# knram06/multigrid_parallel

Hardware: AMD Instinct MI355X
Metric: V-cycles/sec, 513^3 ('512^3') Poisson, V(2,2), fp64 (higher is better)
Workload: dtype f64

## Files before the change

### multigrid_parallel_amd/csrc/mg3d_ctx.hip

```cpp
#include "mg3d_ctx.h"

#include <math.h>
#include <stdarg.h>
#include <stdio.h>
#include <stdlib.h>
#include <string.h>

#include <algorithm>
#include <vector>

static thread_local char g_err[512] = "";

int mg3d_fail(int code, const char *fmt, ...)
{
    va_list ap;
    va_start(ap, fmt);
    vsnprintf(g_err, sizeof g_err, fmt, ap);
    va_end(ap);
    return code;
}
#define fail mg3d_fail

int mg3d_alloc_fail(hipError_t e, const char *who, const char *what)
{
// ... 156 lines not shown
    if (ctx->dep_acc)
        (void)hipFree(ctx->dep_acc);
    if (ctx->dep_max)
        (void)hipFree(ctx->dep_max);
    if (ctx->push_table)
        (void)hipFree(ctx->push_table);
    if (ctx->sort_buf)
        (void)hipFree(ctx->sort_buf);
    for (hipEvent_t e : ctx->io_ev)
        if (e)
            (void)hipEventDestroy(e);
    if (ctx->dz_map)
        (void)hipFree(ctx->dz_map);
    if (ctx->partials)
        (void)hipFree(ctx->partials);
    if (ctx->sumsq)
        (void)hipFree(ctx->sumsq);
    if (ctx->h_sumsq)
        (void)hipHostFree(ctx->h_sumsq);
    resolve_timers(ctx);
    for (hipEvent_t e : ctx->event_pool)
        (void)hipEventDestroy(e);
    if (ctx->stream && ctx->own_stream)
        (void)hipStreamDestroy(ctx->stream);
    delete ctx;
    return MG3D_OK;
}

struct OptionRow {
    const char *key, *env;
    int mode;
    int dflt;
};
static const OptionRow kOptionTable[MG3D_OPT_COUNT] = {
    {"carry", "MG3D_NO_CARRY", 1, 1},
    {"carry_min", "MG3D_CARRY_MIN", 0, 130},
    {"legs", "MG3D_LEGS", 0, 1},
    {"legs_min", "MG3D_LEGS_MIN", 0, 160},
    {"tiny", "MG3D_NO_TINY", 1, 1},
    {"tiny_cycle", "MG3D_NO_TINY_CYCLE", 1, 1},
    {"lu_reduced", "MG3D_LU_REDUCED", 0, 1},
    {"fuse_rst2", "MG3D_FUSE_RST2", 0, -1},
    {"small_max", "MG3D_SMALL_MAX", 0, 129},
    {"fuse_leg_max", "MG3D_FUSE_LEG_MAX", 0, 0},
    {"fuse_up_max", "MG3D_FUSE_UP_MAX", 0, 1 << 20},
    {"sweep_tune", "MG3D_SWEEP_TUNE", 0, -1},
    {"sweep_tune_log", "MG3D_SWEEP_TUNE_LOG", 0, 0},
    {"sweep_ci", "MG3D_SWEEP_CI", 0, 0},
    {"sweep_rj", "MG3D_SWEEP_CFG", 2, 0},
    {"sweep_nw", nullptr, 0, 0},
    {"sweep_pf", nullptr, 0, 0},
    {"d_zero_skip", "MG3D_D_ZERO_SKIP", 0, 1},
    {"zero_front", "MG3D_ZERO_FRONT", 0, 1},
};

void mg3d_options_init(mg3d_options *o)
{
    for (int i = 0; i < MG3D_OPT_COUNT; i++) {
        const OptionRow &r = kOptionTable[i];
        o->v[i] = r.dflt;
        const char *e = r.env ? getenv(r.env) : nullptr;
        if (!e || !e[0])
            continue;
        if (r.mode == 0)
            o->v[i] = atoi(e);
        else if (r.mode == 1)
            o->v[i] = e[0] == '1' ? 0 : 1;
        else {
            int rj = 0, nw = 0, pf = 0;
            if (sscanf(e, "%d,%d,%d", &rj, &nw, &pf) >= 2) {
                o->v[MG3D_OPT_SWEEP_RJ] = rj;
                o->v[MG3D_OPT_SWEEP_NW] = nw;
                o->v[MG3D_OPT_SWEEP_PF] = pf;
            }
            i += 2;
        }
    }
}

int mg3d_option_index(const char *key)
{
    if (key)
        for (int i = 0; i < MG3D_OPT_COUNT; i++)
            if (strcmp(key, kOptionTable[i].key) == 0)
                return i;
    return -1;
}

const char *mg3d_option_key(int index) { return index >= 0 && index < MG3D_OPT_COUNT ? kOptionTable[index].key : nullptr; }

extern "C" const char *mg3d_option_name(int index) { return mg3d_option_key(index); }

static mg3d_ctx *ctx_new(int L, int iters)
{
    mg3d_ctx *ctx = new mg3d_ctx();
    ctx->c = 0;
    ctx->length = 0.;
    ctx->L = L;
    ctx->iters = iters;
    ctx->have_lu = false;
    ctx->sigma = 0.;
    ctx->lu_built = false;
    ctx->lu_h = 0.;
    ctx->periodic = 0;
    ctx->neumann = 0;
    ctx->per_b = nullptr;
// ... 513 lines not shown
{
    if (!ctx || !launches)
        return fail(MG3D_ERR_ARG, "mg3d_ctx_dnone_launches: NULL argument");
    *launches = ctx->dnone_launches;
    return MG3D_OK;
}

extern "C" int mg3d_ctx_sweep_taken(const mg3d_ctx *ctx, int kind, int which, int out[MG3D_SWEEP_TAKEN_FIELDS],
                                    unsigned long long *count, unsigned long long *launches)
{
    static_assert(sizeof(SweepTaken) == MG3D_SWEEP_TAKEN_FIELDS * sizeof(int), "SweepTaken is the MG3D_SWEEP_TAKEN_* fields in order");
    static_assert(MG3D_SWEEP_KIND_LEG_UP + 1 == MG3D_SWEEP_KINDS && MG3D_SWEEP_KIND_PASSES == SWEEP_PASSES &&
                      MG3D_SWEEP_KIND_PASSES_RES == SWEEP_PASSES_RES && MG3D_SWEEP_KIND_TAP == SWEEP_TAP &&
                      MG3D_SWEEP_KIND_LEG_DOWN == SWEEP_LEG_DOWN && MG3D_SWEEP_KIND_LEG_UP == SWEEP_LEG_UP,
                  "MG3D_SWEEP_KIND_* are SweepKind");
    if (!ctx || !out)
        return fail(MG3D_ERR_ARG, "mg3d_ctx_sweep_taken: NULL argument");
    if (kind < 0 || kind >= MG3D_SWEEP_KINDS || which < 0)
        return fail(MG3D_ERR_ARG, "mg3d_ctx_sweep_taken: no such kind, or a negative index");
    const SweepTakenLog &log = ctx->sweep_taken;
    const bool have = which < log.n[kind];
    if (have)
        memcpy(out, &log.e[kind][which].t, sizeof(SweepTaken));
    else
        memset(out, 0, sizeof(SweepTaken));
    if (count)
        *count = have ? log.e[kind][which].count : 0;
    if (launches)
        *launches = log.launches[kind];
    return MG3D_OK;
}

int mg3d_launch_ok(const char *who)
{
    hipError_t e = hipGetLastError();
    if (e != hipSuccess)
        return fail(MG3D_ERR_HIP, "%s: kernel launch failed: %s", who, hipGetErrorString(e));
    return MG3D_OK;
}

static int read_norm(mg3d_ctx *ctx, int slot, double *norm)
{
    if (!norm)
        return MG3D_OK;
    HIPCHK(hipMemcpyAsync(ctx->h_sumsq + slot, ctx->sumsq + slot, sizeof(double), hipMemcpyDeviceToHost,
                          ctx->stream));
    HIPCHK(hipStreamSynchronize(ctx->stream));
    resolve_timers(ctx);
    *norm = sqrt(ctx->h_sumsq[slot]);
    return MG3D_OK;
}

static StageAsk stage_ask(const mg3d_ctx *ctx, int level, int post, int iters, int want_res, bool has_coarse, bool need_norm,
                          bool pro_offered)
{
    const Geom &g = ctx->lv[level].g;
    return StageAsk{g.N, g.nj, post != 0, iters, want_res, has_coarse, need_norm, pro_offered,  true};
}

static int enqueue_stage_step(mg3d_ctx *ctx, int level, int post, const StageStep &st, bool first, int want_res, int slot,
                              Level *coarse, const Level *pro, bool zero_in, bool need_norm)
{
    Level &l = ctx->lv[level];
    SweepLaunch w = mg3d_level_sweep(ctx, l);
    w.kind = st.res ? SWEEP_PASSES_RES : SWEEP_PASSES;
    w.S = st.S;
    w.c1 = post ? 0 : 1;
    if (zero_in && first)
        w.vin = nullptr;
    if (st.res && want_res == 2 && !st.rst)
        w.r = l.f[MG3D_R];
    if (st.res && need_norm)
        w.partials = ctx->partials;
    if (st.rst) {
        w.gc = &coarse->g;
        w.dc = coarse->f[MG3D_D];
    }
    if (st.pro) {
        w.gce = &pro->g;
        w.ec = pro->f[MG3D_U];
    }
    int np;
    {
        StageScope kt(ctx, level, st.S == 4 ? MG3D_K_SWEEP4 : st.S == 2 ? (st.res ? MG3D_K_SWEEP2_RES : MG3D_K_SWEEP2)
                                                                        : MG3D_K_RESIDUAL, true);
        np = k_sweep(ctx->opt, w, ctx->stream);
    }
    if (np < 0)
        return fail(MG3D_ERR_STATE, "fused sweep: no kernel for %d colour passes%s on level %d", st.S,
                    st.res ? " + residual" : "", level);
    if (st.S > 0)
        swap_u(l);
    if (st.res && need_norm)
        k_fold(ctx->partials, np, ctx->sumsq + slot, ctx->stream);
    return MG3D_OK;
}

static int enqueue_smooth_residual(mg3d_ctx *ctx, int level, int post, int iters, int want_res, int slot,
                                    Level *coarse = nullptr, const Level *pro = nullptr, bool zero_in = false,
                                    bool need_norm = true)
{
    Level &l = ctx->lv[level];
    hipStream_t s = ctx->stream;
    if (mg3d_fused(ctx)) {
        const StagePlan plan = mg3d_stage_plan(ctx->opt, stage_ask(ctx, level, post, iters, want_res, coarse != nullptr, need_norm,
                                                                   pro != nullptr));
        for (int k = 0; mg3d_stage_launch(plan, k); k++)
            CHK(enqueue_stage_step(ctx, level, post, *mg3d_stage_launch(plan, k), k == 0, want_res, slot, coarse, pro, zero_in, need_norm));
        return MG3D_OK;
    }
    const int c1 = post ? 0 : 1;
    const LevelOperator A = mg3d_level_operator(ctx, level);
    for (int it = 0; it < 2 * iters; it++) {
        StageScope kt(ctx, level, MG3D_K_COLOUR_PASS, true);
        k_smooth_color(l.g, l.f[MG3D_U], l.f[MG3D_D], A, c1 ^ (it & 1), s);
    }
    if (want_res) {
        StageScope kt(ctx, level, MG3D_K_RESIDUAL, true);
        k_residual(l.g, l.f[MG3D_U], l.f[MG3D_D], A, want_res == 2 ? l.f[MG3D_R] : nullptr, ctx->partials, ctx->sumsq + slot, s);
    }
    return MG3D_OK;
}

static bool pro_fusable(const mg3d_ctx *ctx, int iters, int want_res, int level)
{
    return mg3d_fused(ctx) && mg3d_stage_plan(ctx->opt, stage_ask(ctx, level, 1, iters, want_res, false, true, true)).step[0].pro;
}

static void enqueue_restrict(mg3d_ctx *ctx, int level, bool faces_only = false)
{
    const Level &lev = ctx->lv[level], &lc = ctx->lv[level - 1];
    k_restrict(lev.g, lev.f[MG3D_R], lc.g, lc.f[MG3D_D], mg3d_ctx_bc(ctx), ctx->stream, -1, -1, faces_only);
}

static void enqueue_prolong(mg3d_ctx *ctx, int level)
{
    const Level &lev = ctx->lv[level], &lc = ctx->lv[level - 1];
    k_prolong(lc.g, lc.f[MG3D_U], lev.g, lev.f[MG3D_U], mg3d_ctx_bc(ctx), ctx->stream, -1, -1, mg3d_level_operator(ctx, level).m);
}

static void enqueue_coarse_solve(mg3d_ctx *ctx, const double *rhs = nullptr ,
                                 bool own_values = false )
{
    Level &l0 = ctx->lv[0];
    if (!rhs)
        rhs = l0.f[MG3D_D];
    const int bc = mg3d_ctx_bc(ctx), pin = mg3d_ctx_pinned(ctx);
    const unsigned char *m = mg3d_level_operator(ctx, 0).m;
    if (m || ctx->periodic || (ctx->neumann && pin)) {
        k_coarse_rhs(l0.g, rhs, ctx->per_b, bc, pin, m, (ctx->L == 1 || own_values) ? l0.f[MG3D_U] : nullptr, ctx->stream);
        rhs = ctx->per_b;
    }
    k_lu_solve(ctx->lu, ctx->lu_in, l0.g, rhs, l0.f[MG3D_U], ctx->lu_work, ctx->stream);
    k_per_refresh(l0.g, l0.f[MG3D_U], bc, ctx->stream);
}

static int enqueue_smooth(mg3d_ctx *ctx, int level, int post, int iters)
{
    return enqueue_smooth_residual(ctx, level, post, iters, 0, 0);
// ... 833 lines not shown
```

### multigrid_parallel_amd/csrc/mg3d_dist.hip

```cpp
#include "mg3d_ctx.h"

#include <math.h>
#include <stdio.h>
#include <stdlib.h>
#include <string.h>

#include <rccl/rccl.h>

#include "mg3d_plan.h"

#define fail mg3d_fail
#define HIPCHK(call)                                                                                    \
    do {                                                                                                \
        hipError_t e_ = (call);                                                                         \
        if (e_ != hipSuccess)                                                                           \
            return fail(MG3D_ERR_HIP, "%s failed: %s (%s:%d)", #call, hipGetErrorString(e_), __FILE__, \
                        __LINE__);                                                                      \
    } while (0)
#define NCCLCHK(call)                                                                                    \
    do {                                                                                                 \
        ncclResult_t e_ = (call);                                                                        \
        if (e_ != ncclSuccess)                                                                           \
            return fail(MG3D_ERR_HIP, "%s failed: %s (%s:%d)", #call, ncclGetErrorString(e_), __FILE__, \
                        __LINE__);                                                                       \
// ... 858 lines not shown
                HIPCHK(hipEventRecord(D->ev_now, xs));
                HIPCHK(hipStreamWaitEvent(s, D->ev_now, 0));
            }
        } else
            HIPCHK(hipMemcpyAsync(R.gather, R.coarse->sumsq, sizeof(double), hipMemcpyDeviceToDevice, s));
    }
    hipLaunchKernelGGL(sum_in_order_kernel, dim3(1), dim3(64), 0, s, R.gather, D->P, D->d_norms + slot);
    return MG3D_OK;
}

struct RestrictTarget {
    const Geom *gc;
    double *dc;
    int lo, hi;
};
static void restrict_into(SweepLaunch &w, const RestrictTarget &t)
{
    w.gc = t.gc;
    w.dc = t.dc;
    w.ic_lo = t.lo;
    w.ic_hi = t.hi;
}

struct ProlongSource {
    const Geom *gc;
    const double *ec;
};
static void prolong_from(SweepLaunch &w, const ProlongSource &p)
{
    w.gce = p.gc;
    w.ec = p.ec;
}

struct SlabCycle {
    int slot;
    bool carry_out, legs_out;
    bool carry_in, legs_in;
    bool red_in;
    bool can_legs, can_carry, keep_r;
};

struct Window {
    int lo, hi;
};
static Window slab_window(const SlabLevel &sl, int m)
{
    return Window{sl.own_lo - m < 0 ? 0 : sl.own_lo - m, sl.own_hi + m > sl.lv.g.ni ? sl.lv.g.ni : sl.own_hi + m};
}

static StagePlan dist_stage_plan(mg3d_dist *D, int l, int post, int want_res, bool has_coarse, bool pro_offered)
{
    const Geom &g = SL(D, D->rs[0], l).lv.g;
    return mg3d_stage_plan(D->rs[0].coarse->opt,
                           StageAsk{g.N, g.nj, post != 0, D->nu, want_res, has_coarse, want_res == 1, pro_offered,  false});
}

static SweepLaunch slab_sweep(mg3d_dist *D, size_t ri, int l)
{
    SlabLevel &sl = SL(D, D->rs[ri], l);
    SweepLaunch w = mg3d_level_sweep(D->rs[ri].coarse, sl.lv);
    w.i_lo = w.acc_lo = sl.own_lo;
    w.i_hi = w.acc_hi = sl.own_hi;
    return w;
}

static void swap_u_all(mg3d_dist *D, int l)
{
    for (auto &R : D->rs)
        swap_u(SL(D, R, l).lv);
}

template <class Make, class Done>
static int edge_first(mg3d_dist *D, int l, int margin, int E, const char *what, Make make, Done done)
{
    bool split = D->overlap && D->P > 1;
    std::vector<Window> win;
    for (auto &R : D->rs) {
        win.push_back(slab_window(SL(D, R, l), margin));
        split = split && win.back().hi - win.back().lo >= 2 * E + 2;
    }
    std::vector<int> n_first(D->rs.size());
    for (size_t ri = 0; ri < D->rs.size(); ri++) {
        SweepLaunch w = make(ri, split, -1);
        w.i_lo = win[ri].lo;
        w.i_hi = win[ri].hi;
        w.edge = split ? E : 0;
        n_first[ri] = k_sweep(D->rs[ri].coarse->opt, w, D->stream);
        if (n_first[ri] <= 0)
            return fail(MG3D_ERR_STATE, "slab sweep: no kernel for %s%s on level %d", split ? "the edge windows of " : "", what, l);
        if (!split)
            done(ri, n_first[ri], 0);
    }
    swap_u_all(D, l);
    CHK(start_u_exchange(D, MG3D_XK_HALO_U_NEXT, l));
    for (size_t ri = 0; split && ri < D->rs.size(); ri++) {
        Level &lv = SL(D, D->rs[ri], l).lv;
        SweepLaunch w = make(ri, split, n_first[ri]);
        w.vin = lv.alt;
        w.vout = lv.f[MG3D_U];
        w.i_lo = win[ri].lo + E;
        w.i_hi = win[ri].hi - E;
        const int n_in = k_sweep(D->rs[ri].coarse->opt, w, D->stream);
        if (n_in <= 0)
            return fail(MG3D_ERR_STATE, "slab sweep: no kernel for the interior window of %s on level %d", what, l);
        done(ri, n_first[ri], n_in);
    }
    return MG3D_OK;
// ... 394 lines not shown
```

### multigrid_parallel_amd/csrc/mg3d_internal.h

```cpp
#ifndef MG3D_INTERNAL_H
#define MG3D_INTERNAL_H

#include <hip/hip_runtime.h>
#include <stddef.h>

#include "mg3d.h"

struct Geom {
    int ni, nj, nk;
    int pitch;
    long long plane;
    int ig0;
    int N;
};

static inline int mg3d_pitch_for(int nk) { return (nk + 15) & ~15; }

struct LevelOp {
    double hSq, sixth, invHsq, dg;
};
static inline LevelOp mg3d_level_op(double h, double sigma)
{
    LevelOp op;
    op.hSq = h * h;
    op.dg = 6 + sigma * op.hSq;
    op.sixth = 1. / op.dg;
    op.invHsq = 1. / op.hSq;
    return op;
}

struct LuBand {
    int n;
    int bw;
    double *lcol;
    double *ucol;
    int npad;
    double *diag;
    int fast_div;
    int rot_r;
    double *lrot;
    double *urot;
    int stream_ch;
    double *stream;
    int *in_map;
};

#define MG3D_MAX_PARTIALS 32768

enum {
    MG3D_OPT_CARRY = 0,
    MG3D_OPT_CARRY_MIN,
    MG3D_OPT_LEGS,
    MG3D_OPT_LEGS_MIN,
    MG3D_OPT_TINY,
    MG3D_OPT_TINY_CYCLE,
    MG3D_OPT_LU_REDUCED,
    MG3D_OPT_FUSE_RST2,
    MG3D_OPT_SMALL_MAX,
    MG3D_OPT_FUSE_LEG_MAX,
    MG3D_OPT_FUSE_UP_MAX,
    MG3D_OPT_SWEEP_TUNE,
    MG3D_OPT_SWEEP_TUNE_LOG,
    MG3D_OPT_SWEEP_CI,
    MG3D_OPT_SWEEP_RJ,
    MG3D_OPT_SWEEP_NW,
    MG3D_OPT_SWEEP_PF,
    MG3D_OPT_D_ZERO_SKIP,
    MG3D_OPT_ZERO_FRONT,
    MG3D_OPT_COUNT
};
struct mg3d_options {
    int v[MG3D_OPT_COUNT];
};
void mg3d_options_init(mg3d_options *o);
int mg3d_option_index(const char *key);
const char *mg3d_option_key(int index);

struct LevelOperator {
    LevelOp op;
    double sigma;
    const double *e;
    int bc;
    const unsigned char *m;
    const double *s;
};
static inline int mg3d_bc(int periodic, int neumann) { return periodic | neumann << 3; }

void k_smooth_color(const Geom &g, double *v, const double *d, const LevelOperator &A, int color, hipStream_t s,
                    int i_lo = -1, int i_hi = -1);
void k_residual(const Geom &g, const double *v, const double *d, const LevelOperator &A, double *res, double *partials,
                double *sumsq_out, hipStream_t s, int i_lo = -1, int i_hi = -1, int acc_lo = 0, int acc_hi = -1);
void k_sumsq(const Geom &g, const double *a, double *partials, double *sumsq_out, hipStream_t s);
int k_pcg_apply_dot(const Geom &g, const double *p, const LevelOperator &A, double *q, double *partials, double *dot_out,
                    hipStream_t s);
int k_pcg_update_norm(const Geom &g, int bc, double *x, double *r, const double *p, const double *q, const double *rz,
                      const double *pap, double *partials, double *rr_out, hipStream_t s);
int k_pcg_dot(const Geom &g, int bc, const double *a, const double *b, double *partials, double *dot_out, hipStream_t s);
int k_pcg_direction(const Geom &g, int bc, double *p, const double *z, const double *rz_new, const double *rz_old,
                    hipStream_t s);
int k_wpcg_dot(const Geom &g, int bc, const double *a, const double *b, double *partials, double *dot_out, double *sum_out,
               hipStream_t s);
int k_wpcg_direction(const Geom &g, int bc, double *p, const double *z, const double *rz_new, const double *rz_old,
                     const double *wsum, double W, bool first, hipStream_t s);
int k_wpcg_center(const Geom &g, int bc, double *r, const double *wsum, double W, double *partials, double *rr_out,
                  hipStream_t s);
double k_wpcg_weight_sum(const Geom &g, int bc);
int k_step_rhs(const Geom &g, const double *u0, const double *src, const LevelOperator &A, double a, double c1, double b,
               bool backward_euler, double *d, hipStream_t s);
void k_restrict(const Geom &gf, const double *r, const Geom &gc, double *dc, int bc, hipStream_t s, int ic_lo = -1,
                int ic_hi = -1, bool faces_only = false ,
                const unsigned char *mf = nullptr );
void k_prolong(const Geom &gc, const double *ec, const Geom &gf, double *ef, int bc, hipStream_t s, int if_lo = -1,
               int if_hi = -1, const unsigned char *mf = nullptr );
void k_fill_boundary(const Geom &g, double *v, double h, hipStream_t s);
__host__ __device__ static inline int mg3d_dzero_words(int ni) { return (ni + 31) / 32; }
void k_dzero_scan(const Geom &g, const double *d, unsigned *map, hipStream_t s);
void k_dzero_fill(const Geom &g, unsigned *map, hipStream_t s);
void k_fold(const double *partials, int np, double *out, hipStream_t s);
void k_fold2(const double *pa, int na, const double *pb, int nb, double *out, hipStream_t s);
void k_sweep_set_tune_default(int on);
bool k_sweep_fuse_rst2(const mg3d_options &o, int N);
// ... 2 lines not shown
    SWEEP_PASSES_RES,
    SWEEP_TAP,
    SWEEP_LEG_DOWN,
    SWEEP_LEG_UP
};
struct SweepTaken {
    int S, RES, RJ, NW, PF, ND, DZ, CI, blocks, xcd_remap, ntj, ntk, PRO, RST, DP, TAP, N;
};
#define MG3D_SWEEP_KINDS 5
#define MG3D_SWEEP_TAKEN_KEEP 32
struct SweepTakenLog {
    struct Entry {
        SweepTaken t;
        unsigned long long count;
    };
    Entry e[MG3D_SWEEP_KINDS][MG3D_SWEEP_TAKEN_KEEP];
    int n[MG3D_SWEEP_KINDS];
    unsigned long long launches[MG3D_SWEEP_KINDS];
};
struct SweepLaunch {
    SweepTakenLog *taken = nullptr;
    const Geom *g = nullptr;
    LevelOp op = {};
    const double *vin = nullptr;
    const double *d = nullptr;
    const unsigned *d_zero = nullptr;
    bool d_none = false;
    unsigned long long *d_none_taken = nullptr;
    double *vout = nullptr;
    SweepKind kind = SWEEP_PASSES;
    int S = 0;
    int c1 = 1;
    double *r = nullptr;
    double *partials = nullptr;
    int max_partials = MG3D_MAX_PARTIALS;
    const Geom *gc = nullptr;
    double *dc = nullptr;
    int ic_lo = -1, ic_hi = -1;
    const Geom *gce = nullptr;
    const double *ec = nullptr;
    int i_lo = -1, i_hi = -1, acc_lo = 0, acc_hi = -1, edge = 0;
};
int k_sweep(const mg3d_options &o, const SweepLaunch &w, hipStream_t s);

struct StageAsk {
    int N, nj;
    bool post;
    int iters;
    int want_res;
    bool has_coarse;
    bool need_norm;
    bool pro_offered;
    bool leg4_form;
};
struct StageStep {
    int S;
    int times;
    bool res;
    bool rst;
    bool pro;
    bool last;
};
struct StagePlan {
    int n;
    StageStep step[3];
};
static inline StagePlan mg3d_stage_plan(const mg3d_options &o, const StageAsk &q)
{
    StagePlan p = {0, {}};
    const bool sp = q.post && 2 * q.iters == 4 && q.want_res == 1;
    const int up_max = q.leg4_form && o.v[MG3D_OPT_FUSE_LEG_MAX] > o.v[MG3D_OPT_FUSE_UP_MAX] ? o.v[MG3D_OPT_FUSE_LEG_MAX]
                                                                                              : o.v[MG3D_OPT_FUSE_UP_MAX];
    const bool pro = q.pro_offered && q.post &&
                     (sp || (2 * q.iters == 4 && q.want_res == 0 && (q.nj & 1) != 0 && q.N <= up_max));
    int passes = 2 * q.iters;
    bool done_res = q.want_res == 0;
    while (passes > 0 || !done_res) {
        const int S = (sp && passes >= 2) ? 2 : passes >= 4 ? 4 : passes;
        const bool last = passes - S == 0;
        const bool leg4 = q.leg4_form && S == 4 && q.has_coarse && !q.need_norm && q.want_res != 0 && q.N <= o.v[MG3D_OPT_FUSE_LEG_MAX];
        const bool res = last && q.want_res != 0 && (S != 4 || leg4) && !(S == 2 && q.has_coarse && !k_sweep_fuse_rst2(o, q.N));
        const StageStep st = {S, 1, res, res && q.has_coarse, pro && passes == 2 * q.iters, last};
        StageStep *prev = p.n ? &p.step[p.n - 1] : nullptr;
        if (prev && prev->S == S && !prev->res && !res && !prev->pro && prev->last == last)
            prev->times++;
        else if (p.n < 3)
            p.step[p.n++] = st;
        done_res = done_res || res;
        passes -= S;
    }
    return p;
}

static inline const StageStep *mg3d_stage_launch(const StagePlan &p, int k)
{
    for (int i = 0; i < p.n; k -= p.step[i++].times)
        if (k < p.step[i].times)
            return &p.step[i];
    return nullptr;
}

static inline bool mg3d_run_ahead_policy(const mg3d_options &o, bool legs, int N)
{
    return o.v[legs ? MG3D_OPT_LEGS : MG3D_OPT_CARRY] != 0 && N >= o.v[legs ? MG3D_OPT_LEGS_MIN : MG3D_OPT_CARRY_MIN];
}
static inline bool mg3d_can_run_ahead(const mg3d_options &o, bool legs, int forced, int iters, bool keep_r, int N, int nj)
{
    const bool on = forced >= 0 ? forced != 0 : mg3d_run_ahead_policy(o, legs, N);
    return on && iters == 2 && !keep_r && N > 65 && (nj & 1) != 0;
}
bool k_tiny_fits(const Geom &g, const Geom &gc);
void k_tiny_down(const Geom &g, double *u, const double *d, const double *r, const Geom &gc, double *dc, const LevelOp &op,
                 int iters, hipStream_t s);
void k_tiny_up(const Geom &g, double *u, const double *d, const Geom &gc, const double *ec, const LevelOp &op, int iters,
               hipStream_t s);
bool k_tiny_cycle_fits(const Geom &g, const Geom &gc, const LuBand &lu, const LuBand &lin);
void k_tiny_cycle(const Geom &g, double *u, const double *d, const double *r, const Geom &gc, double *dc, double *xc,
                  const LuBand &lu, const LuBand &lin, const LevelOp &op, int iters, hipStream_t s);
void k_coef_inject(const Geom &gf, const double *ef, const Geom &gc, double *ec, hipStream_t s);
void k_coarse_rhs(const Geom &g, const double *d, double *b, int bc, int pin, const unsigned char *m, const double *ufix,
                  hipStream_t s);
void k_per_refresh(const Geom &g, double *v, int bc, hipStream_t s, const unsigned long long *gate = nullptr);
void k_mask_pack(const Geom &g, unsigned char *m, const mg3d_array &a, int bc, hipStream_t s);
void k_mask_inject(const Geom &gf, const unsigned char *mf, const Geom &gc, unsigned char *mc, hipStream_t s);
void k_mask_refresh(const Geom &g, unsigned char *m, int bc, hipStream_t s);
void k_mask_keep(const Geom &gf, const unsigned char *mf, const Geom &gc, unsigned char *mc, hipStream_t s);
void k_mask_count(const Geom &g, const unsigned char *m, int bc, unsigned long long *out, hipStream_t s);
void k_fmg_interp(const Geom &gc, const double *uc, const Geom &gf, double *uf, int bc, hipStream_t s,
                  const unsigned char *mf = nullptr);
void k_fmg_inject(const Geom &gf, const double *uf, const unsigned char *mf, const Geom &gc, double *uc, int bc, hipStream_t s);
void k_dirichlet_rhs(const Geom &g, const double *u, double *d, int bc, hipStream_t s);
void k_zero_faces(const Geom &g, double *v, int faces, hipStream_t s);
void k_pack(const Geom &g, double *v, const mg3d_array &a, hipStream_t s);
void k_unpack(const Geom &g, const double *v, const mg3d_array &a, hipStream_t s);
// ... 33 lines not shown
```

### multigrid_parallel_amd/csrc/mg3d_sweep.hip

```cpp
#include "mg3d_internal.h"

#include <stdio.h>
#include <stdlib.h>
#include <string.h>

#include <algorithm>
#include <atomic>
#include <map>
#include <type_traits>
#include <mutex>
#include <vector>

#include "mg3d_sweep_kernel.h"

static std::atomic<int> g_sweep_tune_default{1};
void k_sweep_set_tune_default(int on) { g_sweep_tune_default.store(on); }

static int current_device()
{
    int dev = 0;
    (void)hipGetDevice(&dev);
    return dev;
}

static int device_cus()
{
    static std::mutex mu;
    static std::map<int, int> cus;
    const int dev = current_device();
    std::lock_guard<std::mutex> lock(mu);
    auto it = cus.find(dev);
    if (it == cus.end()) {
        hipDeviceProp_t p;
        int n = hipGetDeviceProperties(&p, dev) == hipSuccess ? p.multiProcessorCount : 0;
        if (n <= 0)
            n = 256;
        it = cus.emplace(dev, n).first;
    }
    return it->second;
}

template <int S, int RES, int RJ, int NW, int PF, bool PRO, bool RST, int DP, int TAP, int C1K, bool ND, int ZF>
static bool launch_kernel(const SweepArgs &a, unsigned blocks, hipStream_t s)
{
    if constexpr (ZF != 0) {
        hipLaunchKernelGGL((sweep_kernel<S, RES, RJ, NW, PF, PRO, RST, DP, TAP, C1K, false, false, ZF>), dim3(blocks), dim3(NW * WAVE), 0, s, a);
    } else if constexpr (ND) {
        hipLaunchKernelGGL((sweep_kernel<S, RES, RJ, NW, PF, PRO, RST, DP, TAP, C1K, false, true>), dim3(blocks), dim3(NW * WAVE), 0, s, a);
    } else {
        if constexpr (NW == 8 && ((RJ == 4 && PF == 1) || (RJ == 2 && PF >= 2))) {
            if (a.dz) {
                hipLaunchKernelGGL((sweep_kernel<S, RES, RJ, NW, PF, PRO, RST, DP, TAP, C1K, true>), dim3(blocks), dim3(NW * WAVE), 0, s, a);
                return true;
            }
        }
        hipLaunchKernelGGL((sweep_kernel<S, RES, RJ, NW, PF, PRO, RST, DP, TAP, C1K, false>), dim3(blocks), dim3(NW * WAVE), 0, s, a);
    }
    return false;
}

template <int S, int RES, int RJ, int NW, int PF, bool PRO = false, bool RST = true, int DP = 0, int TAP = -1, int C1K = -1, bool ND = false, int ZF = 0>
static int launch_sweep(const mg3d_options &o, SweepArgs &a, int max_partials, hipStream_t s, SweepTaken *t)
{
    using Sh = SweepShape<S, RES>;
    constexpr int VJ = NW * RJ - 2 * Sh::HJ;
    const Geom &g = a.g;
    if (a.vin == nullptr && ZF != ZF_FRONT && !sweep_tests_input<S, RES, RJ, NW, PF, PRO, RES == 3 ? S / 2 : TAP, ZF>())
        return -1;
    a.ntj = (g.nj + VJ - 1) / VJ;
    auto tiles_for = [&](int vk) { return g.nk <= 2 * WAVE ? 1 : (g.nk - 2 * WAVE + vk - 1) / vk + 1; };
    const int vk_tight = 2 * WAVE - 2 * Sh::HK, vk_line = 2 * WAVE - 16;
    a.vk = (Sh::HK <= 8 && tiles_for(vk_line) <= tiles_for(vk_tight)) ? vk_line : vk_tight;
    a.hk = (2 * WAVE - a.vk) / 2;
    a.ntk = tiles_for(a.vk);
    const int nout = a.i_hi - a.i_lo;
    const int ncu = device_cus();
    const long long T = (long long)a.ntj * a.ntk;
    auto record = [&](bool dz, long long blocks) {
        if (t)
            *t = SweepTaken{S, RES, RJ, NW, PF, (int)ND, (int)dz, a.CI, (int)blocks, a.xcd_remap, a.ntj, a.ntk, (int)PRO, (int)RST, DP, TAP, g.N};
    };
    if (a.edge > 0) {
        if (2 * a.edge > nout || (a.partials && 2 * T > max_partials))
            return -1;
        a.CI = a.edge;
        a.xcd_remap = 2 * T < 64 ? 0 : 2 * T <= ncu ? 1 : 2;
        record(launch_kernel<S, RES, RJ, NW, PF, PRO, RST, DP, TAP, C1K, ND, ZF>(a, (unsigned)(2 * T), s), 2 * T);
        return (int)(2 * T);
    }
    const int ovh = Sh::HI + Sh::ST + (RES == 2 ? 2 : 0) + 1;
    auto model_cost = [&](int ci) -> double {
        const long long blocks = T * ((nout + ci - 1) / ci);
        if (a.partials && blocks > max_partials)
            return -1.;
        const double steps = (double)(ci + ovh);
        const double sat = S >= 4 && (RES == 0 || RES == 3) ? 0.8 : 1.0;
        const double crit = (double)((blocks + ncu - 1) / ncu) * steps, bw = (double)blocks * steps / (sat * ncu);
        return crit > bw ? crit : bw;
    };
    int best_ci = nout;
    double best_cost = 1e30;
    for (int nci = 1; nci <= 64 && nci <= nout; nci++) {
        const int ci = (nout + nci - 1) / nci;
        if (nci > 1 && ci < 2)
            break;
        const double cost = model_cost(ci);
        if (cost < 0)
            break;
        if (cost < best_cost * 0.97) {
            best_cost = cost;
            best_ci = ci;
        }
    }
    int tail_ci = 0;
    if (T < ncu && T * 8 > ncu) {
// ... 163 lines not shown
template <> int dispatch<1, 2>(const mg3d_options &o, SweepArgs &a, SweepCfg c, int max_partials, hipStream_t s, SweepTaken *t)
{
    TRY(1, 2, 4, 8, 1) TRY(1, 2, 4, 8, 2)
    DFLT(1, 2, 4, 8, 1)
}
template <> int dispatch<4, 3>(const mg3d_options &o, SweepArgs &a, SweepCfg c, int max_partials, hipStream_t s, SweepTaken *t)
{
    TRY(4, 3, 4, 8, 1)
    DFLT(4, 3, 4, 8, 1)
}

bool k_sweep_fuse_rst2(const mg3d_options &o, int N)
{
    if (o.v[MG3D_OPT_FUSE_RST2] == 0 || o.v[MG3D_OPT_FUSE_RST2] == 1)
        return o.v[MG3D_OPT_FUSE_RST2] == 1;
    return N >= 130;
}

static bool fill_args(SweepArgs &a, const SweepLaunch &w)
{
    const Geom &g = *w.g;
    a.g = g;
    a.vin = w.vin;
    a.d = w.d;
    a.dz = w.d_zero;
    a.d_none = w.d_none ? 1 : 0;
    a.vout = w.vout;
    a.r = w.r;
    a.partials = w.partials;
    a.hSq = w.op.hSq;
    a.sixth = w.op.sixth;
    a.invHsq = w.op.invHsq;
    a.dg = w.op.dg;
    a.c1 = w.c1;
    a.edge = w.edge;
    a.i_lo = w.i_lo >= 0 ? w.i_lo : 0;
    a.i_hi = w.i_hi >= 0 ? w.i_hi : g.ni;
    a.acc_lo = w.acc_lo;
    a.acc_hi = w.acc_hi < 0 ? g.ni : w.acc_hi;
    a.ec = w.ec;
    a.gce = w.gce ? *w.gce : g;
    a.dc = w.dc;
    if (w.dc) {
        a.gc = *w.gc;
        a.ic_lo = w.ic_lo >= 0 ? w.ic_lo : 0;
        a.ic_hi = w.ic_hi >= 0 ? w.ic_hi : w.gc->ni;
    } else {
        a.gc = g;
        a.ic_lo = a.ic_hi = 0;
    }
    return a.i_hi > a.i_lo;
}

static int sweep_passes(const mg3d_options &o, SweepArgs &a, const SweepLaunch &w, hipStream_t s, SweepTaken *t)
{
    const Geom &g = *w.g;
    const bool tap = w.kind == SWEEP_TAP, residual = w.kind == SWEEP_PASSES_RES;
    const int S = tap ? 4 : w.S, c1 = w.c1, max_partials = w.max_partials;
    const double *const vin = w.vin, *const ec = w.ec;
    double *const dc = w.dc, *const r = w.r, *const partials = w.partials;
    if (dc && (r || partials))
        return -1;
    if (tap) {
        if (S != 4 || dc || ec || r || !partials || residual)
            return -1;
        return dispatch<4, 3>(o, a, opt_cfg(o, {4, 8, 1}), max_partials, s, t);
    }
    if (ec) {
        if (dc || residual || (g.nj & 1) == 0 || c1 != 0)
            return -1;
        if (S == 4)
            return g.N <= o.v[MG3D_OPT_SMALL_MAX] ? launch_sweep<4, 0, 2, 8, 2, true>(o, a, max_partials, s, t)
                                              : launch_sweep<4, 0, 4, 8, 1, true>(o, a, max_partials, s, t);
        if (S == 2)
            return launch_sweep<2, 0, 4, 8, 1, true>(o, a, max_partials, s, t);
        return -1;
    }
    const bool small = g.N <= o.v[MG3D_OPT_SMALL_MAX];
    if (dc && S == 0 && residual)
        return dispatch<0, 2>(o, a, opt_cfg(o, small ? SweepCfg{2, 8, 2} : SweepCfg{4, 8, 1}), max_partials, s, t);
    if (dc && S == 2 && residual)
        return dispatch<2, 2>(o, a, opt_cfg(o, {4, 8, 1}), max_partials, s, t);
    if (dc && S == 1 && residual)
        return dispatch<1, 2>(o, a, opt_cfg(o, {4, 8, 1}), max_partials, s, t);
    if (dc && S == 4 && residual)
        return dispatch<4, 2>(o, a, opt_cfg(o, {2, 8, 2}), max_partials, s, t);
    if (dc)
        return -1;
    if (S == 4 && residual)
        return dispatch<4, 1>(o, a, opt_cfg(o, {6, 4, 2}), max_partials, s, t);
    if (S == 4 && !residual) {
        const bool mid = vin == nullptr && g.N > 65 && g.N <= 300;
        if (vin == nullptr && !w.d_none && !a.dz && o.v[MG3D_OPT_ZERO_FRONT] != 0) {
            const SweepCfg dflt = mid ? SweepCfg{2, 16, 1} : small ? SweepCfg{2, 8, 2} : SweepCfg{4, 8, 1};
            SweepCfg c = opt_cfg(o, dflt);
            if (!((c.rj == 2 && c.nw == 16 && c.pf == 1) || (c.rj == 2 && c.nw == 8 && c.pf == 2) || (c.rj == 4 && c.nw == 8 && c.pf == 1)))
                c = dflt;
            a.c1 = 1 - c1;
            if (c.nw == 16)
                return launch_sweep<3, 0, 2, 16, 1, false, true, 0, -1, -1, false, ZF_FRONT>(o, a, max_partials, s, t);
            if (c.rj == 2)
                return launch_sweep<3, 0, 2, 8, 2, false, true, 0, -1, -1, false, ZF_FRONT>(o, a, max_partials, s, t);
            return launch_sweep<3, 0, 4, 8, 1, false, true, 0, -1, -1, false, ZF_FRONT>(o, a, max_partials, s, t);
        }
        if (vin == nullptr)
            return launch_sweep<4, 0, 2, 16, 1, false, true, 0, -1, -1, false, ZF_MAYBE>(o, a, max_partials, s, t);
        return dispatch<4, 0>(o, a, opt_cfg(o, small ? SweepCfg{2, 8, 2} : SweepCfg{4, 8, 1}), max_partials, s, t);
    }
    if (S == 2 && residual) {
        const SweepCfg c = opt_cfg(o, {4, 8, 1});
        if (!r && c.rj == 4 && c.nw == 8 && (c.pf == 1 || c.pf == 2))
            return c.pf == 1 ? launch_sweep<2, 1, 4, 8, 1, false, false>(o, a, max_partials, s, t)
                             : launch_sweep<2, 1, 4, 8, 2, false, false>(o, a, max_partials, s, t);
        return dispatch<2, 1>(o, a, c, max_partials, s, t);
    }
    if (S == 2 && !residual)
        return dispatch<2, 0>(o, a, opt_cfg(o, small ? SweepCfg{2, 8, 4} : SweepCfg{4, 8, 1}), max_partials, s, t);
    if (S == 0 && residual)
        return dispatch<0, 1>(o, a, opt_cfg(o, {4, 8, 1}), max_partials, s, t);
    return -1;
}


#ifndef MG3D_LEG_UP_RJ
#define MG3D_LEG_UP_RJ 4
#endif
#ifndef MG3D_LEG_DP_UP
#define MG3D_LEG_DP_UP (MG3D_LEG_UP_RJ == 4 ? 0 : 3)
#endif
#ifndef MG3D_LEG_DOWN_RJ
#define MG3D_LEG_DOWN_RJ 4
#endif
#ifndef MG3D_LEG_DP_DOWN3
#define MG3D_LEG_DP_DOWN3 2
#endif
#ifndef MG3D_LEG_ND_PF_DOWN
#define MG3D_LEG_ND_PF_DOWN 1
#endif
#ifndef MG3D_LEG_ND_PF_UP
// ... 124 lines not shown
```

### multigrid_parallel_amd/csrc/mg3d_sweep_kernel.h

```cpp
#ifndef MG3D_SWEEP_KERNEL_H
#define MG3D_SWEEP_KERNEL_H

#include "mg3d_internal.h"

#include <type_traits>

#define WAVE 64

struct SweepArgs {
    Geom g;
    const double *vin;
    const double *d;
    double *vout;
    double *r;
    double *partials;
    double hSq, sixth, invHsq, dg;
    int c1;
    int ntj, ntk;
    int vk, hk;
    int CI;
    int edge;
    int i_lo, i_hi;
    int acc_lo, acc_hi;
    const double *ec;
// ... 62 lines not shown
        return make_double2(x.x, x.y);
    }
}
__device__ __forceinline__ void st_stream(gbytes p, double2 o)
{
    v2d x;
    x.x = o.x;
    x.y = o.y;
#if (MG3D_NT & 2)
    __builtin_nontemporal_store(x, reinterpret_cast<v2d MG3D_GLOBAL *>(p));
#else
    *reinterpret_cast<v2d MG3D_GLOBAL *>(p) = x;
#endif
}
template <int BIT> __device__ __forceinline__ double2 ld_stream(const double *p)
{
    if constexpr ((MG3D_NT & BIT) != 0) {
        const v2d x = __builtin_nontemporal_load(reinterpret_cast<const v2d *>(p));
        return make_double2(x.x, x.y);
    } else {
        return *reinterpret_cast<const double2 *>(p);
    }
}
__device__ __forceinline__ void st_stream(double *p, double2 o)
{
#if (MG3D_NT & 2)
    v2d x;
    x.x = o.x;
    x.y = o.y;
    __builtin_nontemporal_store(x, reinterpret_cast<v2d *>(p));
#else
    *reinterpret_cast<double2 *>(p) = o;
#endif
}

#ifndef MG3D_KERNEL_ATTR
#define MG3D_KERNEL_ATTR
#endif
#ifndef MG3D_STAGE_MAJOR
#define MG3D_STAGE_MAJOR 1
#endif
#ifdef MG3D_DEBUG_BLOCKTIMES
__device__ unsigned long long g_dbg_bt[8][1024];
#ifndef MG3D_DEBUG_BT_COND
#define MG3D_DEBUG_BT_COND (PRO && S == 4 && TAP == 4)
#endif
#endif
enum { ZF_OFF = 0, ZF_FRONT = 1, ZF_MAYBE = 2 };
template <int S, int RES, int RJ, int NW, int PF, bool PRO, int TAPQ, int ZFM> constexpr bool sweep_tests_input()
{
    constexpr bool at_limit = S == 4 && RES == 0 && RJ == 4 && NW == 8 && PF == 2;
    return ZFM == ZF_MAYBE || (ZFM == ZF_OFF && !PRO && TAPQ < 0 && (S == 2 || (S == 4 && RES == 2) || at_limit));
}
template <int S, int RES, int RJ, int NW, int PF, bool PRO, bool RST, int DP, int TAP, int C1K = -1, bool DZ = false, bool ND = false, int ZFM = ZF_OFF>
__global__ void __launch_bounds__(NW *WAVE) MG3D_KERNEL_ATTR sweep_kernel(SweepArgs a)
{
    using Sh = SweepShape<S, RES>;
    constexpr int ST = Sh::ST, HJ = Sh::HJ, HI = Sh::HI;
    constexpr int TAPQ = RES == 3 ? S / 2 : TAP;
    constexpr bool HASTAP = TAPQ >= 0;
    constexpr bool NORM = RES == 1 || HASTAP;
    static_assert(DP >= 0 && DP < ST, "at least one slot of the d window stays in registers");
    static_assert(TAPQ <= S, "tap behind the last pass");
    static_assert(!ND || DP == 0, "no d window: nothing to park");
    static_assert(!ND || !DZ, "no d window: no map to test");
    constexpr bool ZF = ZFM == ZF_FRONT;
    static_assert(ZFM == ZF_OFF || (S == (ZF ? 3 : 4) && RES == 0), "the launch from the zero guess: three passes behind the front, or four");
    static_assert(ZFM == ZF_OFF || (!PRO && !ND && RES == 0 && TAP < 0), "the zero front: plain colour passes on a d that is read");
    static_assert(ZFM == ZF_OFF || (!DZ && DP == 0 && C1K < 0), "the zero front: every plane of d is read, nothing parked, c1 from the launcher");
    constexpr int KV = ST - DP;
    constexpr int TJ = NW * RJ, VJ = TJ - 2 * HJ;
    static_assert(RJ % 2 == 0, "RJ must be even (row parity of a wave's first row)");
    static_assert(VJ > 0 && ST >= 1, "tile too small");
    constexpr int STX = ST > 0 ? ST : 1;
    constexpr bool NDR = ND && RES == 2;

#ifndef MG3D_EX_SINGLE
#define MG3D_EX_SINGLE(S_, RES_, NW_, DP_) ((RES_) == 2 && (NW_) == 8 && (DP_) > 0)
#endif
    constexpr bool EXS = MG3D_EX_SINGLE(S, RES, NW, DP);
    constexpr int EXB = EXS ? 1 : 2;
    __shared__ double ex[EXB][NW][2][STX][WAVE];
    __shared__ double red[NW];
    __shared__ double2 rex[RES == 2 ? EXB : 1][RES == 2 ? NW : 1][RES == 2 ? WAVE : 1];
    constexpr int CO = RES == 2 ? (HJ & 1) : 0;
    constexpr int CRW = PRO ? (NW * RJ) / 2 + 2 : 1, CCW = PRO ? WAVE + 2 : 1;
    __shared__ double cpl[PRO ? 3 : 1][CRW][CCW];
    constexpr bool RPARK = RES == 2 && S > 0 && RJ >= 4 && !ND;
    __shared__ double2 rpark[RPARK ? NW * RJ : 1][RPARK ? WAVE : 1];
    __shared__ double rkpark[RPARK ? NW * RJ : 1][RPARK ? WAVE : 1];
    __shared__ double dpk[DP > 0 ? DP : 1][DP > 0 ? NW * RJ : 1][DP > 0 ? 2 : 1][DP > 0 ? WAVE : 1];

    const Geom &g = a.g;
#ifndef MG3D_UNIFORM_W
#define MG3D_UNIFORM_W 2
#endif
    const int lane = threadIdx.x & (WAVE - 1);
    const int w = (MG3D_UNIFORM_W == 2 || (MG3D_UNIFORM_W == 1 && RES != 0)) ? __builtin_amdgcn_readfirstlane(threadIdx.x / WAVE)
                                                                             : (int)(threadIdx.x / WAVE);
    const int nout = a.i_hi - a.i_lo;
    int vb = blockIdx.x;
    if (a.xcd_remap == 1) {
        const int nblk = gridDim.x, q = nblk >> 3, r = nblk & 7, x = vb & 7, idx = vb >> 3;
        vb = (x < r ? x * (q + 1) : r * (q + 1) + (x - r) * q) + idx;
    }
    int t_lin = 0, off = 0, len = 0;
    {
        const int T = a.ntj * a.ntk;
        const int ch = vb / T;
        int tl = vb - ch * T;
        if (a.xcd_remap == 2) {
            const int r0 = (ch * T) & 7, x = (r0 + tl) & 7;
            int o = 0;
            for (int y = 0; y < x; y++) {
                const int first = (y - r0 + 8) & 7;
                o += first < T ? (T - first + 7) >> 3 : 0;
            }
            tl = o + (tl - ((x - r0 + 8) & 7)) / 8;
        }
        t_lin = tl;
        if (a.edge > 0) {
// ... 638 lines not shown
```

Baseline: 680.6.

## Fuse zero-guess pre-smooth with residual and restriction on large levels

Adds a 'down' stage form. On the pre-smoothing of a level that starts from a zero guess, the four colour passes (three behind the zero front) are fused with the residual and restriction into one sweep kernel instead of separate launches. The zero-front kernel variant is extended to allow RES==2, and a launch path picks RJ/PF configurations for it, gated by a new FUSE_DOWN_MIN option (default 130) so it applies only to large levels. This removes a separate residual/restriction pass over the fine grid, at the cost of a larger halo and more register and shared-memory pressure in the fused kernel.

```diff
diff --git a/multigrid_parallel_amd/csrc/mg3d_ctx.hip b/multigrid_parallel_amd/csrc/mg3d_ctx.hip
--- a/multigrid_parallel_amd/csrc/mg3d_ctx.hip
+++ b/multigrid_parallel_amd/csrc/mg3d_ctx.hip
@@ -232,6 +232,7 @@
     {"sweep_pf", nullptr, 0, 0},
     {"d_zero_skip", "MG3D_D_ZERO_SKIP", 0, 1},
     {"zero_front", "MG3D_ZERO_FRONT", 0, 1},
+    {"fuse_down_min", "MG3D_FUSE_DOWN_MIN", 0, 130},
 };
 
 void mg3d_options_init(mg3d_options *o)
@@ -851,10 +852,11 @@
 }
 
 static StageAsk stage_ask(const mg3d_ctx *ctx, int level, int post, int iters, int want_res, bool has_coarse, bool need_norm,
-                          bool pro_offered)
+                          bool pro_offered, bool zero_in = false)
 {
     const Geom &g = ctx->lv[level].g;
-    return StageAsk{g.N, g.nj, post != 0, iters, want_res, has_coarse, need_norm, pro_offered,  true};
+    return StageAsk{g.N, g.nj, post != 0, iters, want_res, has_coarse, need_norm, pro_offered,  true, zero_in,
+                     true};
 }
 
 static int enqueue_stage_step(mg3d_ctx *ctx, int level, int post, const StageStep &st, bool first, int want_res, int slot,
@@ -903,7 +905,7 @@
     hipStream_t s = ctx->stream;
     if (mg3d_fused(ctx)) {
         const StagePlan plan = mg3d_stage_plan(ctx->opt, stage_ask(ctx, level, post, iters, want_res, coarse != nullptr, need_norm,
-                                                                   pro != nullptr));
+                                                                   pro != nullptr, zero_in));
         for (int k = 0; mg3d_stage_launch(plan, k); k++)
             CHK(enqueue_stage_step(ctx, level, post, *mg3d_stage_launch(plan, k), k == 0, want_res, slot, coarse, pro, zero_in, need_norm));
         return MG3D_OK;
diff --git a/multigrid_parallel_amd/csrc/mg3d_dist.hip b/multigrid_parallel_amd/csrc/mg3d_dist.hip
--- a/multigrid_parallel_amd/csrc/mg3d_dist.hip
+++ b/multigrid_parallel_amd/csrc/mg3d_dist.hip
@@ -934,7 +934,8 @@
 {
     const Geom &g = SL(D, D->rs[0], l).lv.g;
     return mg3d_stage_plan(D->rs[0].coarse->opt,
-                           StageAsk{g.N, g.nj, post != 0, D->nu, want_res, has_coarse, want_res == 1, pro_offered,  false});
+                           StageAsk{g.N, g.nj, post != 0, D->nu, want_res, has_coarse, want_res == 1, pro_offered,  false,  false,
+                                     false});
 }
 
 static SweepLaunch slab_sweep(mg3d_dist *D, size_t ri, int l)
diff --git a/multigrid_parallel_amd/csrc/mg3d_internal.h b/multigrid_parallel_amd/csrc/mg3d_internal.h
--- a/multigrid_parallel_amd/csrc/mg3d_internal.h
+++ b/multigrid_parallel_amd/csrc/mg3d_internal.h
@@ -67,6 +67,7 @@
     MG3D_OPT_SWEEP_PF,
     MG3D_OPT_D_ZERO_SKIP,
     MG3D_OPT_ZERO_FRONT,
+    MG3D_OPT_FUSE_DOWN_MIN,
     MG3D_OPT_COUNT
 };
 struct mg3d_options {
@@ -175,6 +176,8 @@
     bool need_norm;
     bool pro_offered;
     bool leg4_form;
+    bool zero_in;
+    bool down_form;
 };
 struct StageStep {
     int S;
@@ -202,7 +205,10 @@
         const int S = (sp && passes >= 2) ? 2 : passes >= 4 ? 4 : passes;
         const bool last = passes - S == 0;
         const bool leg4 = q.leg4_form && S == 4 && q.has_coarse && !q.need_norm && q.want_res != 0 && q.N <= o.v[MG3D_OPT_FUSE_LEG_MAX];
-        const bool res = last && q.want_res != 0 && (S != 4 || leg4) && !(S == 2 && q.has_coarse && !k_sweep_fuse_rst2(o, q.N));
+        const bool down = q.down_form && q.zero_in && !q.post && 2 * q.iters == 4 && passes == 4 && q.has_coarse && !q.need_norm &&
+                          q.want_res != 0 && o.v[MG3D_OPT_ZERO_FRONT] != 0 && o.v[MG3D_OPT_FUSE_DOWN_MIN] > 0 &&
+                          q.N >= o.v[MG3D_OPT_FUSE_DOWN_MIN] && q.N > o.v[MG3D_OPT_FUSE_LEG_MAX];
+        const bool res = last && q.want_res != 0 && (S != 4 || leg4 || down) && !(S == 2 && q.has_coarse && !k_sweep_fuse_rst2(o, q.N));
         const StageStep st = {S, 1, res, res && q.has_coarse, pro && passes == 2 * q.iters, last};
         StageStep *prev = p.n ? &p.step[p.n - 1] : nullptr;
         if (prev && prev->S == S && !prev->res && !res && !prev->pro && prev->last == last)
diff --git a/multigrid_parallel_amd/csrc/mg3d_sweep.hip b/multigrid_parallel_amd/csrc/mg3d_sweep.hip
--- a/multigrid_parallel_amd/csrc/mg3d_sweep.hip
+++ b/multigrid_parallel_amd/csrc/mg3d_sweep.hip
@@ -59,8 +59,20 @@
     return false;
 }
 
+template <int S, int RES, int RJ, int NW, int PF, bool PRO, bool RST, int DP, int TAP, int C1K, bool ND, int ZF>
+static int launch_sweep_paired(const mg3d_options &o, SweepArgs &a, int max_partials, hipStream_t s, SweepTaken *t);
+
 template <int S, int RES, int RJ, int NW, int PF, bool PRO = false, bool RST = true, int DP = 0, int TAP = -1, int C1K = -1, bool ND = false, int ZF = 0>
 static int launch_sweep(const mg3d_options &o, SweepArgs &a, int max_partials, hipStream_t s, SweepTaken *t)
+{
+    if constexpr (sweep_front_pairing<S, RES, ZF>())
+        return launch_sweep_paired<S, RES, RJ, NW, PF, PRO, RST, DP, TAP, C1K, ND, ZF>(o, a, max_partials, s, t);
+    else
+        return -1;
+}
+
+template <int S, int RES, int RJ, int NW, int PF, bool PRO, bool RST, int DP, int TAP, int C1K, bool ND, int ZF>
+static int launch_sweep_paired(const mg3d_options &o, SweepArgs &a, int max_partials, hipStream_t s, SweepTaken *t)
 {
     using Sh = SweepShape<S, RES>;
     constexpr int VJ = NW * RJ - 2 * Sh::HJ;
@@ -330,6 +342,10 @@
     return a.i_hi > a.i_lo;
 }
 
+#ifndef MG3D_FUSED_DOWN_PF
+#define MG3D_FUSED_DOWN_PF 1
+#endif
+
 static int sweep_passes(const mg3d_options &o, SweepArgs &a, const SweepLaunch &w, hipStream_t s, SweepTaken *t)
 {
     const Geom &g = *w.g;
@@ -361,8 +377,21 @@
         return dispatch<2, 2>(o, a, opt_cfg(o, {4, 8, 1}), max_partials, s, t);
     if (dc && S == 1 && residual)
         return dispatch<1, 2>(o, a, opt_cfg(o, {4, 8, 1}), max_partials, s, t);
-    if (dc && S == 4 && residual)
+    if (dc && S == 4 && residual) {
+        if (vin == nullptr && !w.d_none && !a.dz && o.v[MG3D_OPT_ZERO_FRONT] != 0 && g.N > o.v[MG3D_OPT_FUSE_LEG_MAX]) {
+            const SweepCfg dflt = small ? SweepCfg{2, 8, 2} : SweepCfg{4, 8, MG3D_FUSED_DOWN_PF};
+            SweepCfg c = opt_cfg(o, dflt);
+            if (!((c.rj == 2 && c.nw == 8 && c.pf == 2) || (c.rj == 4 && c.nw == 8 && (c.pf == 1 || c.pf == 2))))
+                c = dflt;
+            a.c1 = 1 - c1;
+            if (c.rj == 2)
+                return launch_sweep<3, 2, 2, 8, 2, false, true, 0, -1, -1, false, ZF_FRONT>(o, a, max_partials, s, t);
+            if (c.pf == 2)
+                return launch_sweep<3, 2, 4, 8, 2, false, true, 0, -1, -1, false, ZF_FRONT>(o, a, max_partials, s, t);
+            return launch_sweep<3, 2, 4, 8, 1, false, true, 0, -1, -1, false, ZF_FRONT>(o, a, max_partials, s, t);
+        }
         return dispatch<4, 2>(o, a, opt_cfg(o, {2, 8, 2}), max_partials, s, t);
+    }
     if (dc)
         return -1;
     if (S == 4 && residual)
diff --git a/multigrid_parallel_amd/csrc/mg3d_sweep_kernel.h b/multigrid_parallel_amd/csrc/mg3d_sweep_kernel.h
--- a/multigrid_parallel_amd/csrc/mg3d_sweep_kernel.h
+++ b/multigrid_parallel_amd/csrc/mg3d_sweep_kernel.h
@@ -138,6 +138,10 @@
     constexpr bool at_limit = S == 4 && RES == 0 && RJ == 4 && NW == 8 && PF == 2;
     return ZFM == ZF_MAYBE || (ZFM == ZF_OFF && !PRO && TAPQ < 0 && (S == 2 || (S == 4 && RES == 2) || at_limit));
 }
+template <int S, int RES, int ZFM> constexpr bool sweep_front_pairing()
+{
+    return ZFM == ZF_OFF || (ZFM == ZF_FRONT && S == 3 && (RES == 0 || RES == 2)) || (ZFM == ZF_MAYBE && S == 4 && RES == 0);
+}
 template <int S, int RES, int RJ, int NW, int PF, bool PRO, bool RST, int DP, int TAP, int C1K = -1, bool DZ = false, bool ND = false, int ZFM = ZF_OFF>
 __global__ void __launch_bounds__(NW *WAVE) MG3D_KERNEL_ATTR sweep_kernel(SweepArgs a)
 {
@@ -151,8 +155,8 @@
     static_assert(!ND || DP == 0, "no d window: nothing to park");
     static_assert(!ND || !DZ, "no d window: no map to test");
     constexpr bool ZF = ZFM == ZF_FRONT;
-    static_assert(ZFM == ZF_OFF || (S == (ZF ? 3 : 4) && RES == 0), "the launch from the zero guess: three passes behind the front, or four");
-    static_assert(ZFM == ZF_OFF || (!PRO && !ND && RES == 0 && TAP < 0), "the zero front: plain colour passes on a d that is read");
+    static_assert(sweep_front_pairing<S, RES, ZFM>(), "the launch from the zero guess: three passes behind the front (alone or with residual + restriction), or four");
+    static_assert(ZFM == ZF_OFF || (!PRO && !ND && TAP < 0), "the zero front: plain colour passes on a d that is read");
     static_assert(ZFM == ZF_OFF || (!DZ && DP == 0 && C1K < 0), "the zero front: every plane of d is read, nothing parked, c1 from the launcher");
     constexpr int KV = ST - DP;
     constexpr int TJ = NW * RJ, VJ = TJ - 2 * HJ;
```

New measurement: 692.7 (median of 6 runs). About the same (+1.8%).
